# grisetti/g2o_frontend

Hardware: AMD Instinct MI355X
Metric: depth-pair alignments/sec (640x480, 10 GN iters) (higher is better)
Workload: dtype f32; 1 GPU; loop-closure batch: 128 independent 640x480 depth pairs per GPU (u16 mm frames resident in HBM; per pair: convert 2 frames + Aligner::align, 10x1 GN iterations); BASELINE configs[3] shard; mode=pairs, pairs_per_gpu=128, total_pairs=128, rows=480, cols=640, sub_frames=64, sub_pairs=64, streams=4, omega_storage=sym6, step_mode=fused, parallelism=independent pairs sharded over 1 GPU(s), RCCL all-gather of result records only

## Files before the change

### g2o_frontend_amd/_lib.py

```python
from __future__ import annotations

import ctypes as C
import os

_HERE = os.path.dirname(os.path.abspath(__file__))
LIB_PATH = os.environ.get("PWN_HIP_LIB", os.path.join(_HERE, "libpwn_hip.so"))
MAX_ITERATIONS = 64

STATUS = {0: "OK", 1: "INVALID_ARGUMENT", 2: "NO_DEVICE", 3: "ALLOCATION", 4: "COPY", 5: "LAUNCH", 6: "CAPACITY"}


class PwnHipError(RuntimeError):
    def __init__(self, code, msg):
        super().__init__(f"pwn_hip status {code} ({STATUS.get(code, '?')}): {msg}")
        self.code = code


class ConverterParams(C.Structure):
    _fields_ = [("K", C.c_float * 9), ("min_distance", C.c_float), ("max_distance", C.c_float),
                ("world_radius", C.c_float), ("min_image_radius", C.c_int), ("max_image_radius", C.c_int),
                ("min_points", C.c_int), ("stats_curvature_threshold", C.c_float),
                ("point_info_curvature_threshold", C.c_float), ("normal_info_curvature_threshold", C.c_float),
                ("point_flat_diag", C.c_float * 3), ("point_nonflat_diag", C.c_float * 3),
                ("normal_flat_diag", C.c_float * 3), ("normal_nonflat_diag", C.c_float * 3),
# ... 142 lines not shown
    "pwn_hip_merge": (_I, [_VP, _VP, _VP, _VP, _F, _F, _I, _I, _F, _F, _F, C.POINTER(_I), _VP]),
    "pwn_hip_merge_clouds": (_I, [_VP, _VP, _VP, _I, _VP, _VP, _F, _F, _I, _I, _VP, _VP, _VP, _VP]),
    "pwn_hip_manifold_image": (_I, [_VP, _I, _VP, _VP, _F, _I, _I, _F, _I, _VP, _VP]),
    "pwn_hip_voxelize": (_I, [_VP, _VP, _F, C.POINTER(_I), _VP]),
    "pwn_hip_cloud_save": (_I, [_VP, _VP, C.c_char_p, _VP, _I, _I]),
    "pwn_hip_cloud_load": (_I, [_VP, _VP, C.c_char_p, _VP]),
    "pwn_hip_last_stage_ms": (_I, [_VP, C.c_char_p, C.POINTER(_F), C.POINTER(_I)]),
    "pwn_hip_set_profiling": (_I, [_VP, _I]),
    "pwn_hip_debug_withhold_carry": (_I, [_VP, _I, _I, _I, _I, _I]),
    "pwn_hip_debug_set_index_shortcut": (_I, [_VP, _I]),
    "pwn_hip_debug_convert_retries": (_I, [_VP, C.POINTER(_I)]),
    "pwn_hip_debug_set_settle_guard": (_I, [_VP, _I]),
    "pwn_hip_debug_projection_fallbacks": (_I, [_VP, C.POINTER(_I)]),
    "pwn_hip_debug_project_pairs": (_I, [_VP, _VP, _I, _VP, _VP, _I, _I, _VP, _VP, C.POINTER(_I)]),
    "pwn_hip_debug_cur_depth_sub_batches": (_I, [_VP, C.POINTER(_I)]),
    "pwn_hip_debug_converter_points": (_I, [_VP, _I, _I, _VP, _F, _VP, _I, _VP]),
    "pwn_hip_debug_stats_from_integral": (_I, [_VP, _VP, _I, _I, _I, _VP, _VP, _VP, _VP, _I]),
    "pwn_hip_debug_stats_from_integral_lean": (_I, [_VP, _VP, _I, _I, _I, _VP, _VP, _VP, _F, _VP, _I]),
    "pwn_hip_debug_front_end": (_I, [_VP, _VP, _VP, _F, _I, _I, _I, _I, _I, _VP, _VP, _VP, _VP, _VP]),
    "pwn_hip_debug_trig_eval": (_I, [_VP, _I, _VP, _VP, _VP, _VP, _VP]),
    "pwn_hip_debug_statistics_eval": (_I, [_VP, _I, _VP, _VP, _VP]),
    "pwn_hip_debug_prior_terms_eval": (_I, [_VP, _I, _VP, _VP, _VP, _VP]),
    "pwn_hip_debug_cloud_set_gaussians": (_I, [_VP, _VP, _I, _VP, _VP, _VP, _VP, _VP]),
    "pwn_hip_debug_cloud_expose_gaussians": (_I, [_VP, _VP, _I]),
    "pwn_hip_debug_set_manifold_chunk": (_I, [_VP, _I]),
    "pwn_hip_debug_set_gaussian_stores": (_I, [_VP, _I]),
    "pwn_hip_measure_hbm": (_I, [_VP, C.c_size_t, _VP, _VP]),
}

_lib = None
# ... 17 lines not shown
```

### g2o_frontend_amd/csrc/pwn_hip_capi.hip

```cpp
#include <cstdlib>
#include "../../include/pwn_hip.h"
#include "../../include/pwn_hip_testing.h"
#include "pwn_buffers.h"
#include "pwn_kernels.h"
#include "pwn_scene_kernels.h"
#include "pwn_stats.h"

#include <algorithm>
#include <chrono>
#include <condition_variable>
#include <functional>
#include <cstddef>
#include <cstdio>
#include <cstring>
#include <map>
#include <mutex>
#include <string>
#include <thread>
#include <type_traits>
#include <vector>

using namespace pwnhip;

namespace {
// ... 87 lines not shown
  void refresh() { front.view(d, sb); d.count = count; }
  hipError_t own(unsigned which) {
    hipError_t e = count.ensure(1);
    if (e == hipSuccess) e = front.ensure(which, (size_t)d.capacity, d.omSym);
    refresh();
    return e;
  }
  void drop_omega_n() { front.OmN.release(); refresh(); }
  void swap_sides() { front.swap(back); refresh(); }
  hipError_t own_back(CloudDev& bd, SceneBuffers& bs) {
    const hipError_t e = back.ensure(kArrCore | front.held(), (size_t)d.capacity, d.omSym);
    bd = d; back.view(bd, bs);
    return e;
  }
  bool plain() const { return front.P3 && front.Nc && front.Om && count && front.held() == kArrCore && back.held() == 0; }
  size_t core_bytes() const { return front.core_bytes() + idximg.cap * sizeof(int); }
  CloudContent content;
  CloudView view() const { CloudView v = { d, sb, content.n, sb.G ? content.n_gauss : 0 }; if (!content.stats) v.d.St = nullptr; return v; }
  DevBuf<int> idximg;
  const pwn_hip_ctx* owner = nullptr;
};

struct pwn_hip_ctx {
  int device = 0;
  hipStream_t stream = nullptr;
  hipStream_t own_stream = nullptr;
  hipStream_t stream2 = nullptr;
  hipStream_t extra[2] = { nullptr, nullptr };
  hipEvent_t fork_ev = nullptr, join_ev = nullptr, join_extra[2] = { nullptr, nullptr };
  hipStream_t copy_stream = nullptr;
  std::vector<hipEvent_t> sync_events;
  hipEvent_t copy_ev = nullptr;
  hipEvent_t foreign_ev = nullptr;
  bool copy_pending = false;
// ... 45 lines not shown
  AsyncConvert* async = nullptr;
  HostBuf<char> flat_hdr_host;
  DevBuf<float> records_ws;
  DevBuf<int> ids_dev;
  DevBuf<int> prior_first_dev; HostBuf<int> prior_first_host;
  DevBuf<PriorHost> priors_dev; HostBuf<PriorHost> priors_host;
  DevBuf<PriorTerms> prior_terms_dev;
  void (*enqueued_cb)(void*) = nullptr; void* enqueued_user = nullptr;
  HostBuf<int> align_fault_host;
  DevBuf<unsigned> zdepth_ws;
  int settle_guard = kSettleGuard;
  int last_align_fault = 0;
  int projection_fallbacks = 0;
  DevBuf<const uint16_t*> cur_raw_dev; HostBuf<const uint16_t*> cur_raw_host;
  int cur_depth_subs = 0;
  DevBuf<float> merge_ws; int merge_planes = 0;
  DevBuf<const float*> plane_ptrs_dev; HostBuf<const float*> plane_ptrs_host;
  DevBuf<DepthCloudDesc> depth_clouds_dev; HostBuf<DepthCloudDesc> depth_clouds_host;
  DevBuf<Mat4> krt_dev; HostBuf<Mat4> krt_host;
  DevBuf<int> merge_counts_dev; HostBuf<int> merge_counts_host;
  DevBuf<float> cloud_weights_ws;
  DevBuf<ManifoldCloud> manifold_dev; HostBuf<ManifoldCloud> manifold_host;
  DevBuf<uint16_t> manifold_img_dev; HostBuf<uint16_t> manifold_img_host;
  int manifold_chunk = kMaxCloudPoints;
};

namespace {

constexpr size_t kCloudPoolBytes = 1ull << 30;

struct PairLaunch { const AlignParams* ap; int nb, sym; int m; hipStream_t st; const PairDesc* pr; unsigned* zd; const CurDepthSrc* cd; };
bool latency_shape(const pwn_hip_ctx* ctx, int nb, int m) { return (long long)nb * m <= ctx->num_cus; }
template <bool SAME_T, bool FULL_H, bool SYM>
void launch_corr_linearize_s(const pwn_hip_ctx* ctx, const PairLaunch& L, unsigned tag, int usePrevTc, int ownRef) {
  if (latency_shape(ctx, L.nb, L.m)) hipLaunchKernelGGL((k_corr_linearize_lat<SAME_T, FULL_H, SYM>), dim3(L.nb, L.m), dim3(kLatBlock), 0, L.st, L.pr, *L.ap, tag, usePrevTc, ownRef);
  else if (L.cd) hipLaunchKernelGGL((k_corr_linearize<SAME_T, FULL_H, SYM, kPixPerThread, true>), dim3(L.nb, L.m), dim3(kAlignBlock), 0, L.st, L.pr, *L.ap, tag, usePrevTc, ownRef, *L.cd);
  else hipLaunchKernelGGL((k_corr_linearize<SAME_T, FULL_H, SYM>), dim3(L.nb, L.m), dim3(kAlignBlock), 0, L.st, L.pr, *L.ap, tag, usePrevTc, ownRef, NoCurDepthSrc());
}
template <bool SAME_T, bool FULL_H>
void launch_corr_linearize(const pwn_hip_ctx* ctx, const PairLaunch& L, unsigned tag, int usePrevTc, int ownRef) {
  if (L.sym) launch_corr_linearize_s<SAME_T, FULL_H, true>(ctx, L, tag, usePrevTc, ownRef);
  else launch_corr_linearize_s<SAME_T, FULL_H, false>(ctx, L, tag, usePrevTc, ownRef);
}

int fail(pwn_hip_ctx* ctx, int code, const std::string& msg) {
  if (ctx) ctx->err = msg;
  g_err = msg;
  return code;
}
void cloud_changes(pwn_hip_ctx* ctx, const pwn_hip_cloud* c) {
  if (ctx && c && (c == ctx->img.ref_cloud || c == ctx->img.cur_cloud)) ctx->img.drop_clouds();
// ... 275 lines not shown
  ctx->desc_cap = 0;
  ctx->img.invalidate();
  const size_t B = (size_t)std::max(n, 16);
  HIPCHK(ctx, ctx->frames_dev.ensure(B), PWN_HIP_ERR_ALLOCATION);
  HIPCHK(ctx, ctx->pairs_dev.ensure(B), PWN_HIP_ERR_ALLOCATION);
  HIPCHK(ctx, ctx->raw_dev.ensure(B), PWN_HIP_ERR_ALLOCATION);
  HIPCHK(ctx, ctx->counts_dev.ensure(B + 1), PWN_HIP_ERR_ALLOCATION);
  HIPCHK(ctx, ctx->state_ws.ensure(B), PWN_HIP_ERR_ALLOCATION);
  HIPCHK(ctx, ctx->frames_host.ensure(B), PWN_HIP_ERR_ALLOCATION);
  HIPCHK(ctx, ctx->pairs_host.ensure(B), PWN_HIP_ERR_ALLOCATION);
  HIPCHK(ctx, ctx->raw_host.ensure(B), PWN_HIP_ERR_ALLOCATION);
  HIPCHK(ctx, ctx->state_host.ensure(B), PWN_HIP_ERR_ALLOCATION);
  HIPCHK(ctx, ctx->counts_host.ensure(B + 1), PWN_HIP_ERR_ALLOCATION);
  HIPCHK(ctx, ctx->cur_raw_dev.ensure(B), PWN_HIP_ERR_ALLOCATION);
  HIPCHK(ctx, ctx->cur_raw_host.ensure(B), PWN_HIP_ERR_ALLOCATION);
  HIPCHK(ctx, ctx->match_dev.ensure(B), PWN_HIP_ERR_ALLOCATION);
  HIPCHK(ctx, ctx->match_host.ensure(B), PWN_HIP_ERR_ALLOCATION);
  HIPCHK(ctx, ctx->stats_dev.ensure(B), PWN_HIP_ERR_ALLOCATION);
  HIPCHK(ctx, ctx->stats_host.ensure(B), PWN_HIP_ERR_ALLOCATION);
  HIPCHK(ctx, ctx->pairstats_dev.ensure(B), PWN_HIP_ERR_ALLOCATION);
  HIPCHK(ctx, ctx->pairstats_host.ensure(B), PWN_HIP_ERR_ALLOCATION);
  ctx->desc_cap = (int)B;
  return PWN_HIP_OK;
}

constexpr int kSinglePassMinFrames = 16;
void launch_stats(const ConvertParams& cp, const FrameDesc* fr, int n, hipStream_t st) {
  const unsigned perFrame = (unsigned)cp.rows * (unsigned)((cp.cols + 255) / 256);
  const unsigned nblk = (n >= 8 ? 8u * (unsigned)((n + 7) / 8) : (unsigned)n) * perFrame;
  hipLaunchKernelGGL(k_stats, dim3(nblk), dim3(256), 0, st, fr, cp, n);
}
int launch_front_end(pwn_hip_ctx* ctx, const ConvertParams& cp, int base, int n, hipStream_t st, bool single_pass, int* fault_out) {
  const FrameDesc* fr = ctx->frames_dev + base;
  if (single_pass) {
    { StageTimer t(ctx, "unproject", st);
      const bool raw = ctx->frames_host[base].raw != nullptr;
      bool aligned = cp.cols % (raw ? 8 : 4) == 0;
      for (int i = 0; i < n && aligned; ++i) {
        const FrameDesc& fd = ctx->frames_host[base + i];
        aligned = ((uintptr_t)(raw ? (const void*)fd.raw : (const void*)fd.depth) & 15u) == 0;
      }
// ... 13 lines not shown
      hipLaunchKernelGGL(k_row_offsets, dim3(n), dim3(1024), 0, st, fr, cp.rows); }
    { StageTimer t(ctx, "integral_rows", st);
      const unsigned epoch = ++ctx->convert_epoch;
      if (epoch == 0) return fail(ctx, PWN_HIP_ERR_LAUNCH, "convert epoch wrapped: recreate the context");
      hipLaunchKernelGGL(k_unproject_integral_rows, dim3(8u * (unsigned)((bands_of(cp.rows) + 7) / 8) * (unsigned)strips_of(cp.cols), n), dim3(256), 0, st, fr, cp,
                         epoch, ctx->fault_dev); }
    { StageTimer t(ctx, "integral_cols", st);
      const bool grouped = cp.lean == kLeanGrouped;
      const dim3 grid = grouped ? dim3((ig_width(0) * cp.cols + kIC_Block - 1) / kIC_Block, kIG_Groups, n)
                                   : dim3((cp.cols + kIC_Block - 1) / kIC_Block, kIntegralChannels, n);
      hipLaunchKernelGGL(k_integral_cols, grid, dim3(kIC_Block), 0, st, fr, cp.rows, cp.cols, (const int*)ctx->fault_dev, fault_out, grouped ? 1 : 0); }
  }
  return PWN_HIP_OK;
}
int launch_convert(pwn_hip_ctx* ctx, const ConvertParams& cp, int base, int n, hipStream_t st, int* fault_out = nullptr) {
  if (int rc = launch_front_end(ctx, cp, base, n, st, n >= kSinglePassMinFrames, fault_out)) return rc;
  { StageTimer t(ctx, "stats", st);
    launch_stats(cp, ctx->frames_dev + base, n, st); }
  HIPCHK(ctx, hipGetLastError(), PWN_HIP_ERR_LAUNCH);
  return PWN_HIP_OK;
}
void fill_frame(pwn_hip_ctx* ctx, int entry, int slot, const float* depth_dev, const CloudDev& cl) {
  FrameDesc& f = ctx->frames_host[entry];
  f.depth = depth_dev; f.raw = nullptr; f.raw_scale = 0.f;
  f.index = ctx->index_ws + (size_t)slot * ctx->N;
  f.interval = ctx->interval_ws + (size_t)slot * ctx->N;
  f.integral = ctx->integral_ws + (size_t)slot * ctx->N * kIntegralChannels;
  f.rowoff = ctx->rowoff_ws + (size_t)slot * ctx->rowoff_slot;
  f.carry = ctx->carry_ws + (size_t)slot * ctx->carry_slot;
  f.cloud = cl;
  f.count_out = nullptr;
}
int cloud_own(pwn_hip_ctx* ctx, pwn_hip_cloud* c, unsigned which) {
  HIPCHK(ctx, c->own(which), PWN_HIP_ERR_ALLOCATION);
  return PWN_HIP_OK;
}
int cloud_replace(pwn_hip_ctx* ctx, pwn_hip_cloud* c, bool keep_stats, bool planes, const OmegaNClasses* cls, const IndexKey* key = nullptr, bool promised = false,
                  bool gauss = false) {
  cloud_changes(ctx, c);
  if (const unsigned which = (keep_stats ? kArrSt : 0u) | (planes ? kArrOmN : 0u) | (gauss ? kArrGauss : 0u)) { if (int rc = cloud_own(ctx, c, which)) return rc; }
  if (!planes && c->d.OmN) { HIPCHK(ctx, hipStreamSynchronize(ctx->stream), PWN_HIP_ERR_LAUNCH); c->drop_omega_n(); }
  if (cls) { std::memcpy(c->d.omN, cls->omN, sizeof(cls->omN)); c->d.clsThr = cls->clsThr; }
  c->content.replace(keep_stats, key, promised);
  return PWN_HIP_OK;
}
void cloud_commit(pwn_hip_cloud* c, int n, const IndexKey* key = nullptr) { if (key) c->content.commit(n, *key); else c->content.commit(n); }
void cloud_commit_with_gaussians(pwn_hip_cloud* c, int n) { c->content.commit_with_gaussians(n); }
int cloud_edit(pwn_hip_ctx* ctx, pwn_hip_cloud* c, int n, bool device_word) {
  c->content.edit(n);
  if (device_word) HIPCHK(ctx, hipMemsetD32Async((hipDeviceptr_t)c->d.count, n, 1, ctx->stream), PWN_HIP_ERR_COPY);
  return PWN_HIP_OK;
}
void stats_unpack(const float* s, float S[16], float ev[3], int* npts) {
  for (int q = 0; q < 16; ++q) S[q] = 0.f;
  for (int r = 0; r < 3; ++r) for (int q = 0; q < 3; ++q) S[r + 4 * q] = s[r + 3 * q];
  S[12] = s[12]; S[13] = s[13]; S[14] = s[14]; S[15] = 1.0f;
  ev[0] = s[9]; ev[1] = s[10]; ev[2] = s[11]; *npts = (int)s[15];
}
// ... 141 lines not shown
  for (int i = 0; i < n; ++i) {
    pwn_hip_cloud* cl = c.clouds[i];
    if (int rc = cloud_replace(ctx, cl, c.keep_stats != 0, false, &cls, &key, cp.hasOffset == 0, gs.on)) return rc;
    job.clouds.push_back(cl);
    if (gs.on) ctx->gauss_host[i] = cl->sb;
    job.src[i] = c.frames[i];
    const void* src = c.frames[i];
    if (job.host_input) src = raw ? (const void*)(ctx->raw_ws + (size_t)slot[i] * ctx->N) : (const void*)(ctx->depth_ws + (size_t)slot[i] * ctx->N);
    float* scaled = sc.step ? ctx->scaled_ws + (size_t)slot[i] * ctx->N : nullptr;
    fill_frame(ctx, i, slot[i], sc.step ? scaled : raw ? nullptr : static_cast<const float*>(src), cl->d);
    if (cl->idximg.cap < N) {
      HIPCHK(ctx, hipStreamSynchronize(ctx->stream), PWN_HIP_ERR_LAUNCH);
      HIPCHK(ctx, cl->idximg.ensure(N), PWN_HIP_ERR_ALLOCATION);
    }
    ctx->frames_host[i].index = cl->idximg;
    if (sc.step) { ctx->scale_host[i].src = src; ctx->scale_host[i].dst = scaled; }
    else if (raw) { ctx->frames_host[i].raw = static_cast<const uint16_t*>(src); ctx->frames_host[i].raw_scale = c.depth_scale; }
  }
  if (sc.step) HIPCHK(ctx, hipMemcpyAsync(ctx->scale_dev, ctx->scale_host, sizeof(ScaleDesc) * n, hipMemcpyHostToDevice, ctx->stream), PWN_HIP_ERR_COPY);
  if (gs.on && n > 0) HIPCHK(ctx, hipMemcpyAsync(ctx->gauss_dev, ctx->gauss_host, sizeof(SceneBuffers) * n, hipMemcpyHostToDevice, ctx->stream), PWN_HIP_ERR_COPY);
  if (direct) for (int i = 0; i < n; ++i) ctx->frames_host[i].count_out = ctx->counts_host + i;
  HIPCHK(ctx, hipMemcpyAsync(ctx->frames_dev, ctx->frames_host, sizeof(FrameDesc) * n, hipMemcpyHostToDevice, ctx->stream), PWN_HIP_ERR_COPY);
  job.cp = cp;
  return PWN_HIP_OK;
}
int convert_stage_frames(pwn_hip_ctx* ctx, const ConvertJob& job, int base, int m, hipStream_t cs) {
  const size_t fbytes = job.srcN * (job.raw ? sizeof(uint16_t) : sizeof(float));
  const int s0 = job.slot[base];
  for (int i = 0; i < m;) {
    int run = 1;
// ... 10 lines not shown
    if (!clouds[i] || !frames[i]) return fail(ctx, PWN_HIP_ERR_INVALID_ARGUMENT, "null frame or cloud");
    if (clouds[i]->d.omSym != clouds[0]->d.omSym) return fail(ctx, PWN_HIP_ERR_INVALID_ARGUMENT, "clouds of one convert batch must share one omega storage (exact9 / sym6)");
  }
  return PWN_HIP_OK;
}
int launch_gaussians(pwn_hip_ctx* ctx, const ConvertJob& job, int base, int m, hipStream_t st) {
  if (m <= 0) return PWN_HIP_OK;
  StageTimer t(ctx, "gaussians", st);
  const dim3 grid((unsigned)((job.N + 255) / 256), (unsigned)m);
  const FrameDesc* fr = ctx->frames_dev + base; const SceneBuffers* sbs = ctx->gauss_dev + base;
  if (ctx->gauss_staged) hipLaunchKernelGGL(k_gaussians_batch<true>, grid, dim3(256), 0, st, fr, sbs, job.cp, job.gauss.iK, job.gauss.fB, job.gauss.alpha);
  else hipLaunchKernelGGL(k_gaussians_batch<false>, grid, dim3(256), 0, st, fr, sbs, job.cp, job.gauss.iK, job.gauss.fB, job.gauss.alpha);
  HIPCHK(ctx, hipGetLastError(), PWN_HIP_ERR_LAUNCH);
  return PWN_HIP_OK;
}
int convert_enqueue(pwn_hip_ctx* ctx, const ConvertJob& job, int base, int m, hipStream_t st, int* fault_out = nullptr) {
  if (job.scale.step) { if (int rc = launch_depth_scale(ctx, job.scale, job.raw, job.depth_scale, base, m, st)) return rc; }
  if (int rc = launch_convert(ctx, job.cp, base, m, st, fault_out)) return rc;
  if (job.gauss.on) return launch_gaussians(ctx, job, base, m, st);
  return PWN_HIP_OK;
}
int convert_commit(pwn_hip_ctx* ctx, ConvertJob& job) {
  if (int rc = counts_apply(ctx, job.clouds.data(), job.n, job.gauss.on)) return rc;
  job.committed = true;
  return PWN_HIP_OK;
}
int convert_finish(pwn_hip_ctx* ctx, ConvertJob& job) {
  if (int rc = sync_counts(ctx, job.n, job.direct)) return rc;
  return convert_commit(ctx, job);
}

// ... 61 lines not shown
  if (int rc = convert_check(ctx, call)) return rc;
  return repeat_once(ctx, kHandoverTimeout, [&](bool) { return convert_batch_once(ctx, call); });
}

int debug_front_end_impl(pwn_hip_ctx* ctx, const ConvertCall& call, bool single_pass, int lean, float* integral_out, int* index_out, int* interval_out,
                         int* rowoff_out) {
  const int n = call.n, rows = call.rows, cols = call.cols; pwn_hip_cloud* const* clouds = call.clouds;
  if (int rc = check_frames_and_clouds(ctx, call.frames, clouds, n)) return rc;
  ctx->stages.clear();
  std::vector<int> slot((size_t)n);
  for (int i = 0; i < n; ++i) slot[i] = i;
  const bool direct = !single_pass && n < kSinglePassMinFrames;
  ConvertJob job;
  if (int rc = convert_prepare(ctx, call, slot, direct, job)) return rc;
  if (job.host_input) { if (int rc = convert_stage_frames(ctx, job, 0, n, ctx->stream)) return rc; }
  if (lean == PWN_HIP_FRONT_END_LEAN_PLANES) job.cp.lean = 1;
  if (!lean) for (int i = 0; i < n; ++i) {
    HIPCHK(ctx, hipMemsetAsync(clouds[i]->d.Nc, 0, sizeof(float4) * (size_t)clouds[i]->d.capacity, ctx->stream), PWN_HIP_ERR_COPY);
    HIPCHK(ctx, hipMemsetAsync(clouds[i]->d.Om, 0, sizeof(float) * clouds[i]->front.Om.cap, ctx->stream), PWN_HIP_ERR_COPY);
  }
  if (int rc = launch_front_end(ctx, job.cp, 0, n, ctx->stream, single_pass, direct ? ctx->counts_host + n : nullptr)) return rc;
  HIPCHK(ctx, hipGetLastError(), PWN_HIP_ERR_LAUNCH);
  const size_t N = job.N, noff = (size_t)rows * (size_t)(single_pass ? strips_of(cols) : 1);
  for (int i = 0; i < n; ++i) {
    const FrameDesc& f = ctx->frames_host[i];
    HIPCHK(ctx, copy_any(integral_out + (size_t)i * N * kIntegralChannels, f.integral, N * kIntegralChannels * sizeof(float), ctx->stream), PWN_HIP_ERR_COPY);
    HIPCHK(ctx, copy_any(index_out + (size_t)i * N, f.index, N * sizeof(int), ctx->stream), PWN_HIP_ERR_COPY);
    HIPCHK(ctx, copy_any(rowoff_out + (size_t)i * noff, f.rowoff, noff * sizeof(int), ctx->stream), PWN_HIP_ERR_COPY);
    if (!lean) HIPCHK(ctx, copy_any(interval_out + (size_t)i * N, f.interval, N * sizeof(int), ctx->stream), PWN_HIP_ERR_COPY);
  }
// ... 384 lines not shown
  return PWN_HIP_OK;
}
int pwn_hip_debug_set_settle_guard(pwn_hip_ctx* ctx, int rounds) {
  if (!ctx) return fail(nullptr, PWN_HIP_ERR_INVALID_ARGUMENT, "null ctx");
  ctx->settle_guard = rounds < 0 ? kSettleGuard : rounds;
  return PWN_HIP_OK;
}
int pwn_hip_debug_projection_fallbacks(pwn_hip_ctx* ctx, int* calls) {
  if (!ctx || !calls) return fail(ctx, PWN_HIP_ERR_INVALID_ARGUMENT, "null argument");
  *calls = ctx->projection_fallbacks;
  return PWN_HIP_OK;
}
int pwn_hip_debug_cur_depth_sub_batches(pwn_hip_ctx* ctx, int* sub_batches) {
  if (!ctx || !sub_batches) return fail(ctx, PWN_HIP_ERR_INVALID_ARGUMENT, "null argument");
  *sub_batches = ctx->cur_depth_subs;
  return PWN_HIP_OK;
}
int pwn_hip_debug_stats_from_integral(pwn_hip_ctx* ctx, const pwn_hip_converter_params* p, int rows, int cols, int nframes, const float* integral,
                                      const int* index_image, const int* interval_image, pwn_hip_cloud* const* clouds, int keep_stats) {
  if (!ctx || !p || !integral || !index_image || !interval_image || !clouds) return fail(ctx, PWN_HIP_ERR_INVALID_ARGUMENT, "null argument");
  return debug_stats_impl(ctx, p, rows, cols, nframes, integral, index_image, interval_image, nullptr, 0.f, clouds, keep_stats);
}
int pwn_hip_debug_stats_from_integral_lean(pwn_hip_ctx* ctx, const pwn_hip_converter_params* p, int rows, int cols, int nframes, const float* integral,
                                           const int* index_image, const void* const* frames, float depth_scale, pwn_hip_cloud* const* clouds, int keep_stats) {
  if (!ctx || !p || !integral || !index_image || !frames || !clouds) return fail(ctx, PWN_HIP_ERR_INVALID_ARGUMENT, "null argument");
  if (depth_scale < 0.f) return fail(ctx, PWN_HIP_ERR_INVALID_ARGUMENT, "negative depth scale");
  return debug_stats_impl(ctx, p, rows, cols, nframes, integral, index_image, nullptr, frames, depth_scale, clouds, keep_stats);
}
int pwn_hip_debug_front_end(pwn_hip_ctx* ctx, const pwn_hip_converter_params* p, const void* const* frames, float depth_scale, int nframes, int rows, int cols,
                            int path, int lean, pwn_hip_cloud* const* clouds, float* integral_out, int* index_out, int* interval_out, int* rowoff_out) {
// ... 925 lines not shown
  HIPCHK(ctx, ctx->prior_first_host.ensure((size_t)n + 1), PWN_HIP_ERR_ALLOCATION);
  HIPCHK(ctx, ctx->priors_dev.ensure(std::max<size_t>(np, 64)), PWN_HIP_ERR_ALLOCATION);
  HIPCHK(ctx, ctx->priors_host.ensure(std::max<size_t>(np, 64)), PWN_HIP_ERR_ALLOCATION);
  HIPCHK(ctx, ctx->prior_terms_dev.ensure(std::max<size_t>(np, 64)), PWN_HIP_ERR_ALLOCATION);
  std::memcpy(ctx->prior_first_host.p, first, sizeof(int) * ((size_t)n + 1));
  for (size_t j = 0; j < np; ++j) ctx->priors_host[j] = prior_host_from(priors[j]);
  HIPCHK(ctx, hipMemcpyAsync(ctx->prior_first_dev, ctx->prior_first_host, sizeof(int) * ((size_t)n + 1), hipMemcpyHostToDevice, st), PWN_HIP_ERR_COPY);
  if (np > 0) HIPCHK(ctx, hipMemcpyAsync(ctx->priors_dev, ctx->priors_host, sizeof(PriorHost) * np, hipMemcpyHostToDevice, st), PWN_HIP_ERR_COPY);
  return PWN_HIP_OK;
}

static int align_check_and_plan(pwn_hip_ctx* ctx, const AlignCall& c, AlignRun& run) {
  if (!ctx || !c.p || !c.refs || !c.curs || (!c.results && !c.records) || c.n < 0) return fail(ctx, PWN_HIP_ERR_INVALID_ARGUMENT, "null argument");
  if (int rc = check_image(ctx, c.p->rows, c.p->cols)) return rc;
  ctx->img.invalidate();
  ctx->last_pairs = 0; ctx->cur_depth_subs = 0;
  if (int rc = check_align_params(ctx, c.p)) return rc;
  if (int rc = start_align_attempt(ctx, run.robust)) return rc;
  run.want_scores = c.scores != nullptr || (c.records && (c.match_records || c.closure_records));
  run.ap = make_align_params(ctx, c.p); run.N = c.p->rows * c.p->cols; run.nb = align_nblocks(run.N);
  ctx->stages.clear();
  run.plan = make_plan(ctx, ctx->sub_pairs, c.n);
  if (int rc = ensure_desc(ctx, c.n)) return rc;
  HIPCHK(ctx, hipEventRecord(ctx->t0, ctx->stream), PWN_HIP_ERR_LAUNCH);
  return PWN_HIP_OK;
}
static int align_describe_pairs(pwn_hip_ctx* ctx, const AlignCall& c, AlignRun& run) {
  const pwn_hip_aligner_params* p = c.p;
  const int n = c.n, sub = run.plan.sub;
  const IndexKey key = index_key(p);
  const bool shortcut = n >= 1 && ctx->index_shortcut && is_identity(forced(p->current_sensor_offset));
// ... 16 lines not shown
    set_last_row(T);
    if (!(shortcut && cu->content.idx_valid && cu->content.idx_key == key)) run.sub_own[i / sub] = 0;
    if (!(shortcut_ref && is_identity(T) && r->content.idx_valid && r->content.idx_key == key)) run.sub_ownref[i / sub] = 0;
    set_pose(st, T, run.ap, KRtCur0);
  }
  for (int i = 0; i < n; ++i) {
    if (run.sub_own[i / sub]) { ctx->pairs_host[i].curidx = c.curs[i]->idximg; run.any_own = true; }
    if (run.sub_ownref[i / sub]) ctx->pairs_host[i].refidx0 = c.refs[i]->idximg;
  }
  if (n > 0) {
    HIPCHK(ctx, hipMemcpyAsync(ctx->pairs_dev, ctx->pairs_host, sizeof(PairDesc) * n, hipMemcpyHostToDevice, ctx->stream), PWN_HIP_ERR_COPY);
    HIPCHK(ctx, hipMemcpyAsync(ctx->state_ws, ctx->state_host, sizeof(PairState) * n, hipMemcpyHostToDevice, ctx->stream), PWN_HIP_ERR_COPY);
    if (c.cur_depth && run.any_own) {
      for (int i = 0; i < n; ++i) ctx->cur_raw_host[i] = static_cast<const uint16_t*>(c.cur_depth->frames[i]);
      HIPCHK(ctx, hipMemcpyAsync(ctx->cur_raw_dev, ctx->cur_raw_host, sizeof(const uint16_t*) * n, hipMemcpyHostToDevice, ctx->stream), PWN_HIP_ERR_COPY);
    }
    if (run.want_scores) HIPCHK(ctx, hipMemsetAsync(ctx->match_dev, 0, sizeof(MatchAcc) * n, ctx->stream), PWN_HIP_ERR_COPY);
  }
  run.priors = n > 0 && c.priors && c.priors->first[n] > 0;
  if (run.priors) { if (int rc = upload_priors(ctx, n, c.priors->first, c.priors->priors, ctx->stream)) return rc; }
  return PWN_HIP_OK;
}
static int align_draw_tags(pwn_hip_ctx* ctx, const AlignCall& c, AlignRun& run) {
  run.tagsPerSub = (unsigned)std::max(1, c.p->outer_iterations);
  const unsigned nsub = (unsigned)((c.n + run.plan.sub - 1) / run.plan.sub);
  if (run.tagsPerSub > kZ32Tag0) return fail(ctx, PWN_HIP_ERR_INVALID_ARGUMENT, "more projections per alignment than z-buffer epoch tags");
  run.rolling = (unsigned long long)nsub * run.tagsPerSub <= kZ32Tag0;
  if (run.rolling && nsub > 0) { if (int rc = take_tags32(ctx, nsub * run.tagsPerSub, &run.tagBase)) return rc; }
  if (!run.rolling) ctx->z32tag_next = 0;
  run.slot0.cur_tag = run.tagBase; run.slot0.ref_tag = run.tagBase - (run.tagsPerSub - 1);
  return PWN_HIP_OK;
}
static int align_enqueue_sub(pwn_hip_ctx* ctx, const AlignCall& c, AlignRun& run, int base, int k) {
  const pwn_hip_aligner_params* p = c.p;
  const int m = std::min(run.plan.sub, c.n - base), N = run.N;
  hipStream_t st = run.plan.stream(k);
  const size_t s0 = (size_t)run.plan.slot0(k);
  CurDepthSrc cd;
  const bool cur_depth = c.cur_depth && run.sub_own[k] && !latency_shape(ctx, run.nb, m);
  if (cur_depth) {
    const ConvertParams& cp = *c.cur_depth->cp;
    cd.raw = ctx->cur_raw_dev + base; cd.scale = c.cur_depth->scale; cd.iKRt = cp.iKRt; cd.hasOffset = cp.hasOffset; cd.offset = cp.offset;
    ++ctx->cur_depth_subs;
  }
  const PairLaunch L = { &run.ap, run.nb, run.omSym, m, st, ctx->pairs_dev + base, run.robust ? ctx->zdepth_ws + s0 * ctx->N : nullptr, cur_depth ? &cd : nullptr };
  int maxcap_ref = 0, maxcap_cur = 0;
  for (int i = 0; i < m; ++i) { maxcap_ref = std::max(maxcap_ref, c.refs[base + i]->d.capacity); maxcap_cur = std::max(maxcap_cur, c.curs[base + i]->d.capacity); }
  const unsigned tag0 = run.rolling ? run.tagBase - (unsigned)k * run.tagsPerSub : kZ32Tag0, lastRefTag = tag0 - (run.tagsPerSub - 1);
  if (!run.rolling) {
    HIPCHK(ctx, hipMemsetAsync(ctx->z32ref_ws + s0 * ctx->N, 0xFF, (size_t)m * ctx->N * 4, st), PWN_HIP_ERR_COPY);
    HIPCHK(ctx, hipMemsetAsync(ctx->z32cur_ws + s0 * ctx->N, 0xFF, (size_t)m * ctx->N * 4, st), PWN_HIP_ERR_COPY);
  }
  if (s0 == 0 || k == 0) {
    run.slot0.pair = base; run.slot0.ref_cloud = c.refs[base]; run.slot0.cur_cloud = c.curs[base];
    run.slot0.cur_tag = tag0; run.slot0.ref_tag = lastRefTag;
  }
  if (c.hooks && c.hooks->pre_sub) { if (int rc = c.hooks->pre_sub(base, m, k, st)) return rc; }
  const bool subPriors = run.priors && c.priors->first[base + m] > c.priors->first[base];
  const PairPriors pp = { ctx->prior_first_dev + base, ctx->prior_terms_dev };
  if (!run.sub_own[k]) {
    StageTimer t(ctx, "project_cur", st);
    if (int rc = launch_project_cur(ctx, L, maxcap_cur, tag0)) return rc; }
  for (int i = 0; i < p->outer_iterations; ++i) {
    const unsigned tag = tag0 - (unsigned)i;
    const int ownRef = (i == 0 && run.sub_ownref[k]) ? 1 : 0;
    if (!ownRef) { StageTimer t(ctx, "project_ref", st);
      if (int rc = launch_project(ctx, L, maxcap_ref, 0, tag)) return rc; }
    for (int j = 0; j < p->inner_iterations; ++j) {
      const bool lastInner = (j == p->inner_iterations - 1);
      { StageTimer t(ctx, "corr_linearize", st);
        if (j == 0) launch_corr_linearize<true, false>(ctx, L, tag, 0, ownRef);
        else launch_corr_linearize<false, false>(ctx, L, tag, 0, ownRef); }
// ... 580 lines not shown
```

### g2o_frontend_amd/csrc/pwn_kernels.h

```cpp
#pragma once

#include <hip/hip_runtime.h>
#include <stdint.h>
#include <type_traits>
#include "pwn_math.h"
#include "pwn_stats.h"

namespace pwnhip {

constexpr int kMaxIter = 64;
constexpr int kIntegralChannels = 10;
constexpr int kAccHtt = 0, kAccHtr = 9, kAccHrr = 18, kAccBt = 27, kAccBr = 30, kAccChi2 = 33, kAccTerms = kAccChi2 + 1;
constexpr int kAccInliers = kAccTerms, kAccCorr = kAccInliers + 1, kAccCand = kAccCorr + 1, kAccN = kAccCand + 1;
constexpr int kPixPerThread = 8;
constexpr int kAlignBlock = 256;
constexpr unsigned long long kZEmpty = ~0ull;
constexpr unsigned kZTag0 = 0xFEu;
constexpr int kZ64IndexBits = 25, kZ64TagShift = 56;
constexpr int kMaxCloudPoints = 1 << kZ64IndexBits;
constexpr int kZIndexBits = 21;
constexpr int kMaxAlignerPoints = 1 << kZIndexBits;
__host__ __device__ __forceinline__ unsigned long long zkey(unsigned tag, float d, int i) {
  return ((unsigned long long)tag << kZ64TagShift) | ((unsigned long long)(__builtin_bit_cast(unsigned, d) & 0x7fffffffu) << kZ64IndexBits) | (unsigned)i;
}
// ... 106 lines not shown
  Mat3 K;
  Mat4 refOffset;
  float minD, maxD;
  float sqDist, normalThr, flatThr, minRatio, maxRatio;
  float maxChi2;
  int robust;
  int settleGuard;
  int mayFreeze;
};

struct CurDepthSrc {
  const uint16_t* const* raw;
  float scale;
  Mat4 iKRt;
  int hasOffset; Mat4 offset;
};
struct NoCurDepthSrc {};

__device__ __forceinline__ float wave_sum(float v) {
#pragma unroll
  for (int off = 32; off > 0; off >>= 1) v += __shfl_xor(v, off, 64);
  return v;
}
template <int CTRL, int ROW_MASK> __device__ __forceinline__ float dpp_f32(float v) {
  return __int_as_float(__builtin_amdgcn_update_dpp(0, __float_as_int(v), CTRL, ROW_MASK, 0xF, false));
}
__device__ __forceinline__ float wave_sum_dpp_lane63(float v) {
  v += dpp_f32<0xB1, 0xF>(v);
  v += dpp_f32<0x4E, 0xF>(v);
  v += dpp_f32<0x141, 0xF>(v);
// ... 1310 lines not shown
    if (SYM) {
      const v3f_raw r0 = *(gptr<const v3f>)(q.curOm + 3u * ci);
      const v3f_raw r1 = *(gptr<const v3f>)(q.curOm + 3u * cap + 3u * ci);
      oP[0] = r0.x; oP[1] = r0.y; oP[2] = r0.z; oP[3] = r0.y; oP[4] = r1.x; oP[5] = r1.y; oP[6] = r0.z; oP[7] = r1.y; oP[8] = r1.z;
    } else {
#pragma unroll
      for (int r3 = 0; r3 < 3; ++r3) {
        const v3f_raw rw = *(gptr<const v3f>)(q.curOm + (size_t)r3 * 3u * cap + 3u * ci);
        oP[3 * r3] = rw.x; oP[3 * r3 + 1] = rw.y; oP[3 * r3 + 2] = rw.z;
      }
    }
  }
  if (linearize_term(rp, rn, make_float3(c.cP.x, c.cP.y, c.cP.z), make_float3(c.cN.x, c.cN.y, c.cN.z), oP, oN, ap.maxChi2, ap.robust, acc))
    cnt[2] += 1.f;
}
template <bool SAME_T, bool FULL_H, bool SYM = false, int PPT = kPixPerThread, bool CUR_DEPTH = false>
__global__ void __launch_bounds__(kAlignBlock, 1) k_corr_linearize(const PairDesc* __restrict__ pairs, AlignParams ap, unsigned tag, int usePrevTc, int ownRefIndex,
                                                                   std::conditional_t<CUR_DEPTH, CurDepthSrc, NoCurDepthSrc> cd) {
  const PairDesc& pd = pairs[blockIdx.y];
  const int N = ap.rows * ap.cols;
  const PairState* stp = pd.state;
  if (ap.mayFreeze && pair_frozen(stp)) { if (!usePrevTc) return; tag = *as_global(&stp->refTag); }
  const Mat4 Tc = uniform_iso_global(as_global((const float*)(usePrevTc ? stp->invTcorrPrev.m : stp->invTcorr.m)));
  const Mat4 Tl = uniform_iso_global(as_global((const float*)stp->invT.m));
  constexpr int kSlots = LdsAcc<FULL_H>::kSlots;
  __shared__ float lacc[kSlots * kAlignBlock];
#pragma unroll
  for (int k = 0; k < kSlots; ++k) lacc[k * kAlignBlock + threadIdx.x] = 0.f;
  const LdsAcc<FULL_H> sums = { &lacc[threadIdx.x] };
  __shared__ float omNtab[27];
  if (threadIdx.x < 27) omNtab[threadIdx.x] = threadIdx.x < 9 ? 0.f : pd.cur.omN[(threadIdx.x - 9) / 9][(threadIdx.x - 9) % 9];
  __syncthreads();
  float cnt[3] = { 0.f, 0.f, 0.f };
  const int nref = min(*as_global((const int*)pd.ref.count), pd.ref.capacity), ncur = min(*as_global((const int*)pd.cur.count), pd.cur.capacity);
  const int pix0 = blockIdx.x * PPT * kAlignBlock + threadIdx.x;
  const PairPtrs q = pair_ptrs(pd);
  gptr<const uint16_t> craw = nullptr;
  int row = 0, col = 0;
  if constexpr (CUR_DEPTH) { craw = as_global(as_global(cd.raw)[blockIdx.y]); row = pix0 / ap.cols; col = pix0 - row * ap.cols; }
  auto load_indices = [&](int j, int& ri, int& ci, unsigned& cr) {
    const int pix = pix0 + j * kAlignBlock;
    ri = -1; ci = -1;
    if (j < PPT && pix < N) {
      ri = ownRefIndex ? q.refidx0[(unsigned)pix] : z32_index(q.zref[(unsigned)pix], tag);
      ci = q.curidx[(unsigned)pix];
      if constexpr (CUR_DEPTH) cr = craw[(unsigned)pix];
    }
  };
  int ri1, ci1, ri2, ci2;
  unsigned cr1 = 0u, cr2 = 0u;
  load_indices(0, ri1, ci1, cr1);
  load_indices(1, ri2, ci2, cr2);
  Candidate nxt;
  candidate_load<CUR_DEPTH>(q, ri1, ci1, nref, ncur, nxt, cr1);
#pragma unroll 1
  for (int j = 0; j < PPT; ++j) {
    Candidate cur = nxt;
    candidate_load<CUR_DEPTH>(q, ri2, ci2, nref, ncur, nxt, cr2);
    load_indices(j + 2, ri2, ci2, cr2);
    if constexpr (CUR_DEPTH) {
      if (cur.valid) {
        const Vec3 p = converter_point(cd.iKRt, cd.hasOffset, cd.offset, col, row, raw_to_metres(cur.craw, cd.scale));
        cur.cP.x = p.x; cur.cP.y = p.y; cur.cP.z = p.z;
      }
    }
    candidate_consume<SAME_T, SYM>(pd, q, ap, Tc, Tl, cur, sums, cnt, omNtab);
    if constexpr (CUR_DEPTH) {
      col += kAlignBlock;
      while (col >= ap.cols) { col -= ap.cols; ++row; }
    }
  }
  float acc[kAccN];
  acc_from_lds<FULL_H>(lacc, threadIdx.x, cnt[0], cnt[1], cnt[2], acc);
  block_reduce_store<FULL_H>(acc, pd.partials + (size_t)blockIdx.x * kAccN, true);
}

constexpr int kLatBlock = 4 * kAlignBlock;
// ... 383 lines not shown
```

### include/pwn_hip_testing.h

```cpp
#ifndef PWN_HIP_TESTING_H
#define PWN_HIP_TESTING_H
#include "pwn_hip.h"
#ifdef __cplusplus
extern "C" {
#endif

int pwn_hip_debug_withhold_carry(pwn_hip_ctx* ctx, int strip, int band, int chain, int rows, int spin_limit);
int pwn_hip_debug_convert_retries(pwn_hip_ctx* ctx, int* retries);

int pwn_hip_debug_set_index_shortcut(pwn_hip_ctx* ctx, int enabled);

int pwn_hip_debug_set_settle_guard(pwn_hip_ctx* ctx, int rounds);
int pwn_hip_debug_projection_fallbacks(pwn_hip_ctx* ctx, int* calls);
int pwn_hip_debug_project_pairs(pwn_hip_ctx* ctx, const pwn_hip_aligner_params* p, int n, pwn_hip_cloud* const* clouds, const float* transforms,
                                int which, int form, int* index_out, float* depth_out, int* gave_up);

int pwn_hip_debug_cur_depth_sub_batches(pwn_hip_ctx* ctx, int* sub_batches);
int pwn_hip_debug_converter_points(const pwn_hip_converter_params* p, int rows, int cols, const uint16_t* raw, float depth_scale, const int* index_image,
                                   int capacity, float* points);

int pwn_hip_debug_stats_from_integral(pwn_hip_ctx* ctx, const pwn_hip_converter_params* p, int rows, int cols, int nframes, const float* integral,
                                      const int* index_image, const int* interval_image, pwn_hip_cloud* const* clouds, int keep_stats);
int pwn_hip_debug_stats_from_integral_lean(pwn_hip_ctx* ctx, const pwn_hip_converter_params* p, int rows, int cols, int nframes, const float* integral,
                                           const int* index_image, const void* const* frames, float depth_scale, pwn_hip_cloud* const* clouds,
                                           int keep_stats);
enum { PWN_HIP_FRONT_END_LATENCY = 0, PWN_HIP_FRONT_END_SINGLE_PASS = 1 };
enum { PWN_HIP_FRONT_END_LEAN_OFF = 0, PWN_HIP_FRONT_END_LEAN_PLANES = 1, PWN_HIP_FRONT_END_LEAN_GROUPED = 2 };
int pwn_hip_debug_front_end(pwn_hip_ctx* ctx, const pwn_hip_converter_params* p, const void* const* frames, float depth_scale, int nframes, int rows,
                            int cols, int path, int lean, pwn_hip_cloud* const* clouds, float* integral_out, int* index_out, int* interval_out,
                            int* rowoff_out);
int pwn_hip_debug_trig_eval(pwn_hip_ctx* ctx, int n, const float* y, const float* x, float* theta, float* cos_theta, float* sin_theta);
int pwn_hip_debug_statistics_eval(pwn_hip_ctx* ctx, int n, const float* H, const float* T, float* out);
// ... 16 lines not shown
```

Baseline: 13330 alignments/s.

## Rebuild current-frame point indices from per-strip offsets inside linearize kernel

```diff
diff --git a/g2o_frontend_amd/_lib.py b/g2o_frontend_amd/_lib.py
--- a/g2o_frontend_amd/_lib.py
+++ b/g2o_frontend_amd/_lib.py
@@ -180,6 +180,7 @@
     "pwn_hip_debug_projection_fallbacks": (_I, [_VP, C.POINTER(_I)]),
     "pwn_hip_debug_project_pairs": (_I, [_VP, _VP, _I, _VP, _VP, _I, _I, _VP, _VP, C.POINTER(_I)]),
     "pwn_hip_debug_cur_depth_sub_batches": (_I, [_VP, C.POINTER(_I)]),
+    "pwn_hip_debug_strip_index_sub_batches": (_I, [_VP, C.POINTER(_I)]),
     "pwn_hip_debug_converter_points": (_I, [_VP, _I, _I, _VP, _F, _VP, _I, _VP]),
     "pwn_hip_debug_stats_from_integral": (_I, [_VP, _VP, _I, _I, _I, _VP, _VP, _VP, _VP, _I]),
     "pwn_hip_debug_stats_from_integral_lean": (_I, [_VP, _VP, _I, _I, _I, _VP, _VP, _VP, _F, _VP, _I]),
diff --git a/g2o_frontend_amd/csrc/pwn_hip_capi.hip b/g2o_frontend_amd/csrc/pwn_hip_capi.hip
--- a/g2o_frontend_amd/csrc/pwn_hip_capi.hip
+++ b/g2o_frontend_amd/csrc/pwn_hip_capi.hip
@@ -125,10 +125,12 @@
     return e;
   }
   bool plain() const { return front.P3 && front.Nc && front.Om && count && front.held() == kArrCore && back.held() == 0; }
-  size_t core_bytes() const { return front.core_bytes() + idximg.cap * sizeof(int); }
+  size_t core_bytes() const { return front.core_bytes() + (idximg.cap + stripoff.cap) * sizeof(int); }
   CloudContent content;
   CloudView view() const { CloudView v = { d, sb, content.n, sb.G ? content.n_gauss : 0 }; if (!content.stats) v.d.St = nullptr; return v; }
   DevBuf<int> idximg;
+  DevBuf<int> stripoff; bool stripoff_filled = false;
+  bool strip_table() const { return content.idx_valid && stripoff_filled && stripoff; }
   const pwn_hip_ctx* owner = nullptr;
 };
 
@@ -204,6 +206,8 @@
   int projection_fallbacks = 0;
   DevBuf<const uint16_t*> cur_raw_dev; HostBuf<const uint16_t*> cur_raw_host;
   int cur_depth_subs = 0;
+  DevBuf<const int*> cur_strip_dev; HostBuf<const int*> cur_strip_host;
+  int strip_index_subs = 0;
   DevBuf<float> merge_ws; int merge_planes = 0;
   DevBuf<const float*> plane_ptrs_dev; HostBuf<const float*> plane_ptrs_host;
   DevBuf<DepthCloudDesc> depth_clouds_dev; HostBuf<DepthCloudDesc> depth_clouds_host;
@@ -224,7 +228,8 @@
 template <bool SAME_T, bool FULL_H, bool SYM>
 void launch_corr_linearize_s(const pwn_hip_ctx* ctx, const PairLaunch& L, unsigned tag, int usePrevTc, int ownRef) {
   if (latency_shape(ctx, L.nb, L.m)) hipLaunchKernelGGL((k_corr_linearize_lat<SAME_T, FULL_H, SYM>), dim3(L.nb, L.m), dim3(kLatBlock), 0, L.st, L.pr, *L.ap, tag, usePrevTc, ownRef);
-  else if (L.cd) hipLaunchKernelGGL((k_corr_linearize<SAME_T, FULL_H, SYM, kPixPerThread, true>), dim3(L.nb, L.m), dim3(kAlignBlock), 0, L.st, L.pr, *L.ap, tag, usePrevTc, ownRef, *L.cd);
+  else if (L.cd && L.cd->strips) hipLaunchKernelGGL((k_corr_linearize<SAME_T, FULL_H, SYM, kPixPerThread, true, true>), dim3(L.nb, L.m), dim3(kAlignBlock), 0, L.st, L.pr, *L.ap, tag, usePrevTc, ownRef, *L.cd);
+  else if (L.cd) hipLaunchKernelGGL((k_corr_linearize<SAME_T, FULL_H, SYM, kPixPerThread, true>),dim3(L.nb, L.m), dim3(kAlignBlock), 0, L.st, L.pr, *L.ap, tag, usePrevTc, ownRef, *L.cd);
   else hipLaunchKernelGGL((k_corr_linearize<SAME_T, FULL_H, SYM>), dim3(L.nb, L.m), dim3(kAlignBlock), 0, L.st, L.pr, *L.ap, tag, usePrevTc, ownRef, NoCurDepthSrc());
 }
 template <bool SAME_T, bool FULL_H>
@@ -530,6 +535,8 @@
   HIPCHK(ctx, ctx->counts_host.ensure(B + 1), PWN_HIP_ERR_ALLOCATION);
   HIPCHK(ctx, ctx->cur_raw_dev.ensure(B), PWN_HIP_ERR_ALLOCATION);
   HIPCHK(ctx, ctx->cur_raw_host.ensure(B), PWN_HIP_ERR_ALLOCATION);
+  HIPCHK(ctx, ctx->cur_strip_dev.ensure(B), PWN_HIP_ERR_ALLOCATION);
+  HIPCHK(ctx, ctx->cur_strip_host.ensure(B), PWN_HIP_ERR_ALLOCATION);
   HIPCHK(ctx, ctx->match_dev.ensure(B), PWN_HIP_ERR_ALLOCATION);
   HIPCHK(ctx, ctx->match_host.ensure(B), PWN_HIP_ERR_ALLOCATION);
   HIPCHK(ctx, ctx->stats_dev.ensure(B), PWN_HIP_ERR_ALLOCATION);
@@ -541,6 +548,7 @@
 }
 
 constexpr int kSinglePassMinFrames = 16;
+bool single_pass_launch(int n) { return n >= kSinglePassMinFrames; }
 void launch_stats(const ConvertParams& cp, const FrameDesc* fr, int n, hipStream_t st) {
   const unsigned perFrame = (unsigned)cp.rows * (unsigned)((cp.cols + 255) / 256);
   const unsigned nblk = (n >= 8 ? 8u * (unsigned)((n + 7) / 8) : (unsigned)n) * perFrame;
@@ -584,7 +592,7 @@
   return PWN_HIP_OK;
 }
 int launch_convert(pwn_hip_ctx* ctx, const ConvertParams& cp, int base, int n, hipStream_t st, int* fault_out = nullptr) {
-  if (int rc = launch_front_end(ctx, cp, base, n, st, n >= kSinglePassMinFrames, fault_out)) return rc;
+  if (int rc = launch_front_end(ctx, cp, base, n, st, single_pass_launch(n), fault_out)) return rc;
   { StageTimer t(ctx, "stats", st);
     launch_stats(cp, ctx->frames_dev + base, n, st); }
   HIPCHK(ctx, hipGetLastError(), PWN_HIP_ERR_LAUNCH);
@@ -612,6 +620,7 @@
   if (!planes && c->d.OmN) { HIPCHK(ctx, hipStreamSynchronize(ctx->stream), PWN_HIP_ERR_LAUNCH); c->drop_omega_n(); }
   if (cls) { std::memcpy(c->d.omN, cls->omN, sizeof(cls->omN)); c->d.clsThr = cls->clsThr; }
   c->content.replace(keep_stats, key, promised);
+  c->stripoff_filled = false;
   return PWN_HIP_OK;
 }
 void cloud_commit(pwn_hip_cloud* c, int n, const IndexKey* key = nullptr) { if (key) c->content.commit(n, *key); else c->content.commit(n); }
@@ -783,6 +792,15 @@
       HIPCHK(ctx, cl->idximg.ensure(N), PWN_HIP_ERR_ALLOCATION);
     }
     ctx->frames_host[i].index = cl->idximg;
+    if (cp.hasOffset == 0 && c.cols % kIR_Cols == 0) {
+      const size_t words = (size_t)c.rows * (size_t)strips_of(c.cols);
+      if (cl->stripoff.cap < words) {
+        HIPCHK(ctx, hipStreamSynchronize(ctx->stream), PWN_HIP_ERR_LAUNCH);
+        HIPCHK(ctx, cl->stripoff.ensure(words), PWN_HIP_ERR_ALLOCATION);
+      }
+      ctx->frames_host[i].rowoff = cl->stripoff;
+      cl->stripoff_filled = true;
+    }
     if (sc.step) { ctx->scale_host[i].src = src; ctx->scale_host[i].dst = scaled; }
     else if (raw) { ctx->frames_host[i].raw = static_cast<const uint16_t*>(src); ctx->frames_host[i].raw_scale = c.depth_scale; }
   }
@@ -823,7 +841,9 @@
   HIPCHK(ctx, hipGetLastError(), PWN_HIP_ERR_LAUNCH);
   return PWN_HIP_OK;
 }
+void no_strip_tables(const ConvertJob& job, int base, int m) { for (int i = 0; i < m; ++i) job.clouds[(size_t)(base + i)]->stripoff_filled = false; }
 int convert_enqueue(pwn_hip_ctx* ctx, const ConvertJob& job, int base, int m, hipStream_t st, int* fault_out = nullptr) {
+  if (!single_pass_launch(m)) no_strip_tables(job, base, m);
   if (job.scale.step) { if (int rc = launch_depth_scale(ctx, job.scale, job.raw, job.depth_scale, base, m, st)) return rc; }
   if (int rc = launch_convert(ctx, job.cp, base, m, st, fault_out)) return rc;
   if (job.gauss.on) return launch_gaussians(ctx, job, base, m, st);
@@ -915,6 +935,7 @@
   ConvertJob job;
   if (int rc = convert_prepare(ctx, call, slot, direct, job)) return rc;
   if (job.host_input) { if (int rc = convert_stage_frames(ctx, job, 0, n, ctx->stream)) return rc; }
+  if (!single_pass) no_strip_tables(job, 0, n);
   if (lean == PWN_HIP_FRONT_END_LEAN_PLANES) job.cp.lean = 1;
   if (!lean) for (int i = 0; i < n; ++i) {
     HIPCHK(ctx, hipMemsetAsync(clouds[i]->d.Nc, 0, sizeof(float4) * (size_t)clouds[i]->d.capacity, ctx->stream), PWN_HIP_ERR_COPY);
@@ -1329,6 +1350,11 @@
 int pwn_hip_debug_cur_depth_sub_batches(pwn_hip_ctx* ctx, int* sub_batches) {
   if (!ctx || !sub_batches) return fail(ctx, PWN_HIP_ERR_INVALID_ARGUMENT, "null argument");
   *sub_batches = ctx->cur_depth_subs;
+  return PWN_HIP_OK;
+}
+int pwn_hip_debug_strip_index_sub_batches(pwn_hip_ctx* ctx, int* sub_batches) {
+  if (!ctx || !sub_batches) return fail(ctx, PWN_HIP_ERR_INVALID_ARGUMENT, "null argument");
+  *sub_batches = ctx->strip_index_subs;
   return PWN_HIP_OK;
 }
 int pwn_hip_debug_stats_from_integral(pwn_hip_ctx* ctx, const pwn_hip_converter_params* p, int rows, int cols, int nframes, const float* integral,
@@ -2284,7 +2310,7 @@
   if (!ctx || !c.p || !c.refs || !c.curs || (!c.results && !c.records) || c.n < 0) return fail(ctx, PWN_HIP_ERR_INVALID_ARGUMENT, "null argument");
   if (int rc = check_image(ctx, c.p->rows, c.p->cols)) return rc;
   ctx->img.invalidate();
-  ctx->last_pairs = 0; ctx->cur_depth_subs = 0;
+  ctx->last_pairs = 0; ctx->cur_depth_subs = 0; ctx->strip_index_subs = 0;
   if (int rc = check_align_params(ctx, c.p)) return rc;
   if (int rc = start_align_attempt(ctx, run.robust)) return rc;
   run.want_scores = c.scores != nullptr || (c.records && (c.match_records || c.closure_records));
@@ -2331,6 +2357,8 @@
     if (c.cur_depth && run.any_own) {
       for (int i = 0; i < n; ++i) ctx->cur_raw_host[i] = static_cast<const uint16_t*>(c.cur_depth->frames[i]);
       HIPCHK(ctx, hipMemcpyAsync(ctx->cur_raw_dev, ctx->cur_raw_host, sizeof(const uint16_t*) * n, hipMemcpyHostToDevice, ctx->stream), PWN_HIP_ERR_COPY);
+      for (int i = 0; i < n; ++i) ctx->cur_strip_host[i] = c.curs[i]->stripoff;
+      HIPCHK(ctx, hipMemcpyAsync(ctx->cur_strip_dev, ctx->cur_strip_host, sizeof(const int*) * n, hipMemcpyHostToDevice, ctx->stream), PWN_HIP_ERR_COPY);
     }
     if (run.want_scores) HIPCHK(ctx, hipMemsetAsync(ctx->match_dev, 0, sizeof(MatchAcc) * n, ctx->stream), PWN_HIP_ERR_COPY);
   }
@@ -2358,6 +2386,7 @@
   if (cur_depth) {
     const ConvertParams& cp = *c.cur_depth->cp;
     cd.raw = ctx->cur_raw_dev + base; cd.scale = c.cur_depth->scale; cd.iKRt = cp.iKRt; cd.hasOffset = cp.hasOffset; cd.offset = cp.offset;
+    cd.strips = nullptr; cd.minD = cp.minD; cd.maxD = cp.maxD;
     ++ctx->cur_depth_subs;
   }
   const PairLaunch L = { &run.ap, run.nb, run.omSym, m, st, ctx->pairs_dev + base, run.robust ? ctx->zdepth_ws + s0 * ctx->N : nullptr, cur_depth ? &cd : nullptr };
@@ -2373,6 +2402,11 @@
     run.slot0.cur_tag = tag0; run.slot0.ref_tag = lastRefTag;
   }
   if (c.hooks && c.hooks->pre_sub) { if (int rc = c.hooks->pre_sub(base, m, k, st)) return rc; }
+  if (cur_depth) {
+    bool tables = true;
+    for (int i = 0; i < m && tables; ++i) tables = c.curs[base + i]->strip_table();
+    if (tables) { cd.strips = ctx->cur_strip_dev + base; ++ctx->strip_index_subs; }
+  }
   const bool subPriors = run.priors && c.priors->first[base + m] > c.priors->first[base];
   const PairPriors pp = { ctx->prior_first_dev + base, ctx->prior_terms_dev };
   if (!run.sub_own[k]) {
diff --git a/g2o_frontend_amd/csrc/pwn_kernels.h b/g2o_frontend_amd/csrc/pwn_kernels.h
--- a/g2o_frontend_amd/csrc/pwn_kernels.h
+++ b/g2o_frontend_amd/csrc/pwn_kernels.h
@@ -144,6 +144,8 @@
   float scale;
   Mat4 iKRt;
   int hasOffset; Mat4 offset;
+  const int* const* strips;
+  float minD, maxD;
 };
 struct NoCurDepthSrc {};
 
@@ -1484,7 +1486,7 @@
   if (linearize_term(rp, rn, make_float3(c.cP.x, c.cP.y, c.cP.z), make_float3(c.cN.x, c.cN.y, c.cN.z), oP, oN, ap.maxChi2, ap.robust, acc))
     cnt[2] += 1.f;
 }
-template <bool SAME_T, bool FULL_H, bool SYM = false, int PPT = kPixPerThread, bool CUR_DEPTH = false>
+template <bool SAME_T, bool FULL_H, bool SYM = false, int PPT = kPixPerThread, bool CUR_DEPTH = false, bool STRIP_IDX = false>
 __global__ void __launch_bounds__(kAlignBlock, 1) k_corr_linearize(const PairDesc* __restrict__ pairs, AlignParams ap, unsigned tag, int usePrevTc, int ownRefIndex,
                                                                    std::conditional_t<CUR_DEPTH, CurDepthSrc, NoCurDepthSrc> cd) {
   const PairDesc& pd = pairs[blockIdx.y];
@@ -1508,13 +1510,35 @@
   gptr<const uint16_t> craw = nullptr;
   int row = 0, col = 0;
   if constexpr (CUR_DEPTH) { craw = as_global(as_global(cd.raw)[blockIdx.y]); row = pix0 / ap.cols; col = pix0 - row * ap.cols; }
+  static_assert(CUR_DEPTH || !STRIP_IDX, "the strip ranks are counted on the depths of the depth source");
+  constexpr int kWaves = kAlignBlock / 64;
+  static_assert((PPT + 1) * kWaves <= 64, "the strips of a tile and of the turn of look-ahead behind it are lanes of one wave");
+  int tileoff = -1;
+  const int wave = __builtin_amdgcn_readfirstlane(threadIdx.x >> 6);
+  if constexpr (STRIP_IDX) {
+    const unsigned lane = lane_id(), strip = blockIdx.x * (PPT * kWaves) + lane;
+    if (lane < (unsigned)(PPT * kWaves) && strip < ((unsigned)N >> 6)) tileoff = as_global(as_global(cd.strips)[blockIdx.y])[strip];
+  }
   auto load_indices = [&](int j, int& ri, int& ci, unsigned& cr) {
     const int pix = pix0 + j * kAlignBlock;
     ri = -1; ci = -1;
     if (j < PPT && pix < N) {
       ri = ownRefIndex ? q.refidx0[(unsigned)pix] : z32_index(q.zref[(unsigned)pix], tag);
-      ci = q.curidx[(unsigned)pix];
+      if constexpr (!STRIP_IDX) ci = q.curidx[(unsigned)pix];
       if constexpr (CUR_DEPTH) cr = craw[(unsigned)pix];
+    }
+  };
+  auto cur_index = [&](int j, int ci, unsigned& cr) {
+    if constexpr (STRIP_IDX) {
+      const int off = __builtin_amdgcn_readlane(tileoff, kWaves * j + wave);
+      const float d = raw_to_metres(cr, cd.scale);
+      const bool valid = off >= 0 && depth_in_range(d, cd.minD, cd.maxD);
+      const unsigned long long bal = __builtin_amdgcn_ballot_w64(valid);
+      const int idx = (int)__builtin_amdgcn_mbcnt_hi((unsigned)(bal >> 32), __builtin_amdgcn_mbcnt_lo((unsigned)bal, (unsigned)off));
+      cr = __float_as_uint(d);
+      return valid ? idx : -1;
+    } else {
+      return ci;
     }
   };
   int ri1, ci1, ri2, ci2;
@@ -1522,15 +1546,18 @@
   load_indices(0, ri1, ci1, cr1);
   load_indices(1, ri2, ci2, cr2);
   Candidate nxt;
+  ci1 = cur_index(0, ci1, cr1);
   candidate_load<CUR_DEPTH>(q, ri1, ci1, nref, ncur, nxt, cr1);
 #pragma unroll 1
   for (int j = 0; j < PPT; ++j) {
     Candidate cur = nxt;
+    ci2 = cur_index(j + 1, ci2, cr2);
     candidate_load<CUR_DEPTH>(q, ri2, ci2, nref, ncur, nxt, cr2);
     load_indices(j + 2, ri2, ci2, cr2);
     if constexpr (CUR_DEPTH) {
       if (cur.valid) {
-        const Vec3 p = converter_point(cd.iKRt, cd.hasOffset, cd.offset, col, row, raw_to_metres(cur.craw, cd.scale));
+        const float d = STRIP_IDX ? __uint_as_float(cur.craw) : raw_to_metres(cur.craw, cd.scale);
+        const Vec3 p = converter_point(cd.iKRt, cd.hasOffset, cd.offset, col, row, d);
         cur.cP.x = p.x; cur.cP.y = p.y; cur.cP.z = p.z;
       }
     }
diff --git a/include/pwn_hip_testing.h b/include/pwn_hip_testing.h
--- a/include/pwn_hip_testing.h
+++ b/include/pwn_hip_testing.h
@@ -16,6 +16,7 @@
                                 int which, int form, int* index_out, float* depth_out, int* gave_up);
 
 int pwn_hip_debug_cur_depth_sub_batches(pwn_hip_ctx* ctx, int* sub_batches);
+int pwn_hip_debug_strip_index_sub_batches(pwn_hip_ctx* ctx, int* sub_batches);
 int pwn_hip_debug_converter_points(const pwn_hip_converter_params* p, int rows, int cols, const uint16_t* raw, float depth_scale, const int* index_image,
                                    int capacity, float* points);
 
```

Measured after the change: 13520 alignments/s (median of 6 runs). 1.4% higher.
